# DINT-NSDI24/DINT

Hardware: AMD Instinct MI355X
Metric: Mtxn/s + p50/p99 batch latency, TATP (higher is better)
Workload: dtype u64

## Files before the change

### dint_amd/_lib.py

```python
from __future__ import annotations

import ctypes as C
import os

HERE = os.path.dirname(os.path.abspath(__file__))
LIB_PATH = os.environ.get("DINT_LIB_PATH") or os.path.join(HERE, "libdint.so")

ABI_VERSION = 5
FLAG_KV_ROUNDS, FLAG_COPY_STREAMS, FLAG_LOCK_SAME_KEY, FLAG_KV_NO_HOT, FLAG_INPUTS_READY = 1, 2, 4, 8, 16
MICRO_BATCH = 65536

SYMBOLS = [
    "dint_engine_create", "dint_engine_destroy", "dint_msg_size", "dint_last_error", "dint_submit",
    "dint_submit_device", "dint_sync", "dint_load_rows", "dint_populate", "dint_hash_size", "dint_dump_rows",
    "dint_read_locks", "dint_read_log", "dint_get_stats", "dint_reset", "dint_snapshot", "dint_restore",
    "dint_home_shard", "dint_bench_rand64", "dint_timing_enable", "dint_timing_read", "dint_kv_trace_read",
    "dint_submit_async", "dint_wait", "dint_alloc_pinned", "dint_free_pinned", "dint_engine_stream", "dint_max_pass",
    "dint_stream_wait", "dint_stream_signal", "dint_route_pack", "dint_route_unpack", "dint_submit_segments",
    "dint_log_drain", "dint_refuse", "dint_route_pack_multi", "dint_route_unpack_multi", "dint_bench_access", "dint_selftest",
    "dint_submit_segments_multi", "dint_submit_device_ahead", "dint_submit_segments_multi_ahead",
    "dint_log_drain_device", "dint_log_apply_device", "dint_state_digest", "dint_state_diff", "dint_state_repair",
    "dint_state_export", "dint_state_import", "dint_state_rehash", "dint_state_stats",
]
REHASH_DROP_LOCKS = 1
# ... 132 lines not shown
        "dint_route_pack_multi": (C.c_int, [C.POINTER(RouteItem), u32, u64, u64, vp]),
        "dint_route_unpack_multi": (C.c_int, [C.POINTER(RouteItem), u32, u64, vp]),
        "dint_submit_segments": (C.c_int, [vp, vp, u32, u32, u64, vp, u64, vp]),
        "dint_submit_segments_multi": (C.c_int, [C.POINTER(SegmentsItem), u32, vp]),
        "dint_submit_segments_multi_ahead": (C.c_int, [C.POINTER(SegmentsItem), u32, C.POINTER(SegmentsItem), vp]),
        "dint_log_drain": (i64, [vp, vp, u64, C.POINTER(u64)]),
        "dint_refuse": (C.c_int, [u32, vp, u32, vp]),
        "dint_log_drain_device": (i64, [vp, vp, u64, C.POINTER(u64), vp]),
        "dint_log_apply_device": (C.c_int, [vp, vp, u64, u32, C.POINTER(ApplyStats)]),
        "dint_state_digest": (C.c_int, [vp, C.POINTER(TableDigest), u32, vp]),
        "dint_state_diff": (i64, [vp, vp, vp, u64, C.POINTER(DiffStats), vp]),
        "dint_state_repair": (C.c_int, [vp, vp, u64, C.POINTER(RepairStats), vp]),
        "dint_state_export": (C.c_int, [vp, u32, u32, vp, u64, C.POINTER(ImageStats), vp]),
        "dint_state_import": (C.c_int, [vp, vp, u64, C.POINTER(ImageStats), vp]),
        "dint_state_rehash": (C.c_int, [vp, C.POINTER(vp), u32, u32, C.POINTER(RehashStats), vp]),
        "dint_state_stats": (C.c_int, [vp, C.POINTER(TableStats), u32, vp]),
        "dint_log_classify_host": (C.c_int, [vp, u64, vp, vp]),
        "dint_state_row_hash_host": (u64, [u64, u32, u32, vp, u32]),
        "dint_state_digest_host": (C.c_int, [u32, vp, vp, vp, u32, u64, C.POINTER(TableDigest)]),
        "dint_state_diff_host": (i64, [u32, u64, u32, vp, vp, vp, u64, vp, vp, vp, u64, vp, u64, C.POINTER(DiffStats)]),
        "dint_state_image_check_host": (C.c_int, [vp, u64]),
        "dint_state_stats_image_host": (C.c_int, [vp, u64, C.POINTER(TableStats), u32]),
        "dint_state_rehash_place_host": (i64, [vp, u64, u64, u32, u32, vp, vp, vp]),
    }
    for name, (res, args) in sig.items():
        f = getattr(L, name)
        f.restype, f.argtypes = res, args
    _lib = L
    return L


def check(rc: int) -> int:
    if rc < 0:
        raise DintError(f"dint error {rc}: {load().dint_last_error().decode(errors='replace')}")
    return rc
```

### dint_amd/csrc/dint_kv.h

```cpp
#pragma once
#include <cstdlib>
#include <utility>
#include <vector>

#include "dint_kernels.h"
#include "dint_kv_core.h"
#include "state_image.h"

#define DINT_KV_MAX_TABLES 5
#define DINT_KV_CTL_BYTES (64 + 24 * KV_NLISTS)
#define DINT_KV_TRACE_WORDS ((size_t)DINT_KV_PMAX * 16 + 16 * 8192)
#define DINT_KV_LOAD_OP 0xF0u

struct kv_dev {
  kv_tab tab[DINT_KV_MAX_TABLES];
  dint_mod mod[DINT_KV_MAX_TABLES];
  dint_mod lockmod[DINT_KV_MAX_TABLES];
  uint32_t gk_base[DINT_KV_MAX_TABLES];
  uint32_t n_tables;
  uint32_t shard_index, shard_count;
  uint32_t same_key;
};

struct dint_kv_knobs {
  uint32_t coarse_load = 512;
  uint32_t cap = 0;
  uint32_t lcap = 1024;
  uint32_t cap_mult = 64;
  uint32_t rpt = 0;
  uint32_t no_bm = 0;
  uint32_t hot_min = 0;
  uint32_t no_split = 0;
  uint32_t split_min = 65;
  uint32_t split_target = 384;
  uint32_t one_big_kernel = 0;
  uint32_t workers = 96;
  uint32_t part_first = 0;
  uint32_t sb_split_min = 65;
  uint32_t sb_npmax = 128;
  uint32_t sb_workers = 130;
  uint32_t sb_late_grid = 32;
  uint32_t residency = 0;
  uint32_t no_fuse = 0;
  uint32_t no_ahead = 0;
  uint32_t late_grid = 8;
  uint32_t exp_no_late = 0;
  uint32_t late_fat = 0;
  uint32_t late_big = 0;
};

struct dint_kv {
  uint32_t workload = 0;
  uint32_t n_tables = 0;
  uint32_t val_size = 0;
  int force_rounds = 0;
  uint64_t hash_size[DINT_KV_MAX_TABLES] = {0, 0, 0, 0, 0};
  kv_dev h{};
  kv_dev *d_dev = nullptr;
  uint8_t *d_ctl = nullptr;
  uint64_t *d_trace = nullptr;
  size_t entry_bytes[DINT_KV_MAX_TABLES] = {0, 0, 0, 0, 0};
  dint_kv_knobs knobs;
};

static inline uint32_t dint_kv_cap_mult() {
  const char *v = getenv("DINT_KV_CAP_MULT");
  const unsigned long m = v && *v ? strtoul(v, nullptr, 10) : 64ul;
  return (uint32_t)(m < 2 ? 2 : m > 256 ? 256 : m);
}
int dint_kv_create(dint_kv *kv, uint32_t workload, uint64_t n_rows, dint_shard shard, uint32_t pool_entries = 0,
                   uint32_t flags = 0);
void dint_kv_destroy(dint_kv *kv);
std::vector<std::pair<void *, size_t>> dint_kv_regions(dint_kv *kv);
// ... 132 lines not shown
```

### dint_amd/csrc/k_kv.hip

```cpp
#include "k_kv_dev.h"

dint_kv_fmt dint_kv_format(uint32_t workload) {
  switch (workload) {
    case DINT_WL_STORE: return {53, 0, 0xFFFFFFFFu, 1, 9, 49, 40};
    case DINT_WL_TATP: return {55, 1, 2, 3, 11, 51, 40};
    default: return {23, 1, 2, 3, 11, 19, 8};
  }
}


static inline uint32_t kv_pick_coarse(uint32_t n, uint32_t load) {
  uint64_t c = ((uint64_t)n + load - 1) / load;
  if (c < 1) c = 1;
  if (c > DINT_KV_CMAX) c = DINT_KV_CMAX;
  return (uint32_t)c;
}
static uint32_t kv_env(const char *name, uint32_t dflt) {
  const char *v = getenv(name);
  return v && *v ? (uint32_t)strtoul(v, nullptr, 10) : dflt;
}
static dint_kv_knobs kv_read_knobs() {
  dint_kv_knobs k;
  k.coarse_load = std::min(8192u, std::max(64u, kv_env("DINT_KV_COARSE_LOAD", KVB_T)));
  k.cap = kv_env("DINT_KV_CAP", 0);
  k.lcap = std::min(KVR_LCAP, kv_env("DINT_KV_LCAP", KVR_LCAP));
  k.cap_mult = dint_kv_cap_mult();
  k.rpt = kv_env("DINT_KV_RPT", 0);
  k.no_bm = kv_env("DINT_KV_NO_BM", 0);
  k.hot_min = kv_env("DINT_KV_HOT_MIN", 0);
  k.no_split = kv_env("DINT_KV_NO_SPLIT", 0);
  k.split_min = std::max(65u, kv_env("DINT_KV_SPLIT_MIN", 65u));
  k.split_target = std::min(448u, std::max(8u, kv_env("DINT_KV_SPLIT_TARGET", 384u)));
  k.one_big_kernel = kv_env("DINT_KV_ONE_BIG_KERNEL", 0);
  k.no_ahead = kv_env("DINT_KV_NO_AHEAD", 0);
  k.no_fuse = kv_env("DINT_KV_NO_FUSE", 0);
  k.sb_split_min = kv_env("DINT_KV_SB_SPLIT_MIN", 65u);
  k.sb_late_grid = std::max(1u, std::min(KVB_GRID, kv_env("DINT_KV_SB_LATE_GRID", 32u)));
  k.sb_npmax = std::max(2u, std::min(KSB_NPMAX, kv_env("DINT_KV_SB_NPMAX", 128u)));
  k.sb_workers = kv_env("DINT_KV_SB_WORKERS", k.sb_npmax + 2u);
  if (k.sb_workers) k.sb_workers = std::max(k.sb_workers, k.sb_npmax + 2u);
  k.workers = std::min(1024u, std::max(KVR_NPMAX + 2u, kv_env("DINT_KV_WORKERS", KVW_GRID)));
  k.part_first = kv_env("DINT_KV_PART_FIRST", 0) & 1u;
  k.late_grid = std::min(KVB_GRID, std::max(1u, kv_env("DINT_KV_LATE_GRID", 8u)));
  k.late_big = kv_env("DINT_KV_LATE_BIG", 0);
  k.exp_no_late = kv_env("DINT_EXP_NO_LATE", 0);
  k.late_fat = kv_env("DINT_KV_LATE_FAT", 0);
// ... 104 lines not shown
  kv_multi_args M, N;
  memset(&M, 0, sizeof M);
  uint32_t n_total = 0;
  for (uint32_t k = 0; k < n_eng; k++) n_total += p[k].n;
  const uint32_t rpt = kv_pick_rpt(n_total, p[0].kv->knobs);
  for (uint32_t k = 0; k < n_eng; k++) kv_fill_pass(M.e[k], p[k].d_req, p[k].d_rep, p[k].n, *p[k].kv, p[k].log, p[k].s, 0, p[k].view, KV_TB * rpt);
  uint32_t next_rpt = 0;
  if (next) {
    uint32_t nmax = 0;
    for (uint32_t k = 0; k < n_eng; k++) nmax = std::max(nmax, next[k].n);
    next_rpt = kv_pick_rpt_ahead(nmax, p[0].kv->knobs);
    memset(&N, 0, sizeof N);
    for (uint32_t k = 0; k < n_eng; k++) {
      dint_scratch sn = next[k].s;
      sn.kvs.pass_no = p[k].s.kvs.pass_no + 1;
      sn.pass_seq = p[k].s.pass_seq + 1 >= 0x3FFFFFFFu ? 1u : p[k].s.pass_seq + 1;
      kv_fill_pass(N.e[k], next[k].d_req, next[k].d_rep, next[k].n, *next[k].kv, next[k].log, sn, 0, next[k].view, KVB_T * next_rpt);
    }
  }
  launch_kv_dispatch(p[0].kv->workload, M, n_eng, rpt, st, nullptr, p[0].kv->knobs, part_done, next ? &N : nullptr, next_rpt);
}
bool dint_kv_multi_ahead_ok(const dint_kv &kv) { return dint_kv_ahead_ok(kv, 0) && !kv.knobs.no_fuse; }

__global__ void __launch_bounds__(256)
k_home_kv(const uint8_t *__restrict__ req, uint32_t n, const kv_dev *__restrict__ kv, dint_kv_fmt f,
          uint8_t *__restrict__ home) {
  const uint32_t i = blockIdx.x * 256u + threadIdx.x;
  if (i >= n) return;
  const uint8_t *m = req + (size_t)i * f.msg;
  const uint32_t table = f.table == 0xFFFFFFFFu ? 0 : m[f.table];
  if (table >= kv->n_tables) { home[i] = 0xFF; return; }
  const uint64_t g = dint_fastmod(dint_hash_key(ld_u64(m + f.key)), kv->mod[table]);
  home[i] = (uint8_t)(g % (kv->shard_count ? kv->shard_count : 1));
}
void dint_launch_home_kv(const void *d_req, uint32_t n, const dint_kv &kv, uint8_t *d_home, hipStream_t st) {
  if (n == 0) return;
  hipLaunchKernelGGL(k_home_kv, dim3((n + 255) / 256), dim3(256), 0, st, (const uint8_t *)d_req, n, kv.d_dev,
                     dint_kv_format(kv.workload), d_home);
}

int dint_kv_create(dint_kv *kv, uint32_t workload, uint64_t n_rows, dint_shard shard, uint32_t pool_entries,
                   uint32_t flags) {
  *kv = dint_kv();
  kv->workload = workload;
  kv->h.same_key = (workload == DINT_WL_TATP && (flags & DINT_FLAG_LOCK_SAME_KEY)) ? 1 : 0;
  uint64_t hs[DINT_KV_MAX_TABLES] = {0, 0, 0, 0, 0};
// ... 27 lines not shown
    if (hs[t] == 0) hs[t] = 1;
    kv->hash_size[t] = hs[t];
    kv_tab &tb = kv->h.tab[t];
    tb.n_local = (hs[t] + count - 1) / count;
    const uint64_t pool = pool_entries ? pool_entries : tb.n_local / 4 + 4096;
    if (pool > 0xFFFFFFF0ull || gk + tb.n_local > 0xFFFFFFF0ull) return DINT_EINVAL;
    tb.pool_cap = (uint32_t)pool;
    tb.stride = stride;
    tb.val_size = kv->val_size;
    kv->entry_bytes[t] = (size_t)(tb.n_local + tb.pool_cap) * stride;
    if (hipMalloc((void **)&tb.entries, kv->entry_bytes[t]) != hipSuccess) return DINT_ENOMEM;
    if (hipMemset(tb.entries, 0, kv->entry_bytes[t]) != hipSuccess) return DINT_EHIP;
    if (hipMalloc((void **)&tb.pool_next, (size_t)tb.pool_cap * 4) != hipSuccess) return DINT_ENOMEM;
    hipMemset(tb.pool_next, 0, (size_t)tb.pool_cap * 4);
    uint8_t *ctl = kv->d_ctl + DINT_KV_CTL_BYTES * t;
    tb.pool_top = (uint32_t *)ctl;
    tb.free_head = (unsigned long long *)(ctl + 64);
    tb.pend_head = (unsigned long long *)(ctl + 64 + 8 * KV_NLISTS);
    kv->h.mod[t] = dint_make_mod(hs[t]);
    kv->h.lockmod[t] = dint_make_mod(4 * hs[t]);
    kv->h.gk_base[t] = (uint32_t)gk;
    gk += tb.n_local;
  }
  kv->knobs = kv_read_knobs();
  {
    int dev = 0;
    (void)hipGetDevice(&dev);
    const int res = workload == DINT_WL_STORE ? kv_piece_residency<DINT_WL_STORE>(dev)
                    : workload == DINT_WL_TATP ? kv_piece_residency<DINT_WL_TATP>(dev) : kv_piece_residency<DINT_WL_SMALLBANK>(dev);
    kv->knobs.residency = (uint32_t)std::max(res, 0);
    if (workload == DINT_WL_SMALLBANK) {
      if (res < (int)(KSB_NPMAX + 2u + 32u)) kv->knobs.sb_split_min = 0;
    } else {
      if (res < 2 * (int)(KVR_NPMAX + 2u)) kv->knobs.no_split = 1;
      kv->knobs.workers = std::max(KVR_NPMAX + 2u, std::min(kv->knobs.workers, (uint32_t)std::max(res, 0) / 2u));
    }
  }
  if (getenv("DINT_KV_TRACE")) {
    if (hipMalloc((void **)&kv->d_trace, (size_t)DINT_KV_TRACE_WORDS * 8) != hipSuccess) return DINT_ENOMEM;
    hipMemset(kv->d_trace, 0, (size_t)DINT_KV_TRACE_WORDS * 8);
  }
  if (hipMalloc((void **)&kv->d_dev, sizeof(kv_dev)) != hipSuccess) return DINT_ENOMEM;
  if (hipMemcpy(kv->d_dev, &kv->h, sizeof(kv_dev), hipMemcpyHostToDevice) != hipSuccess) return DINT_EHIP;
  return 0;
}

void dint_kv_destroy(dint_kv *kv) {
// ... 133 lines not shown
```

### dint_amd/csrc/k_kv_dev.h

```cpp
#pragma once
#include <algorithm>
#include <cstdlib>
#include <cstring>
#include <utility>
#include <vector>

#include "../../include/dint_abi.h"
#include "dint_kv.h"
#define KVB_SORT_INLINE
#include "dint_bins.h"

template <int WL> struct Fmt;
template <> struct Fmt<DINT_WL_STORE> {
  static constexpr uint32_t MSG = 53, TYPE = 0, KEY = 1, VAL = 9, VER = 49, VS = 40;
  static constexpr bool HAS_TABLE = false;
  static constexpr uint32_t TABLE = 0;
};
template <> struct Fmt<DINT_WL_TATP> {
  static constexpr uint32_t MSG = 55, TYPE = 1, KEY = 3, VAL = 11, VER = 51, VS = 40;
  static constexpr bool HAS_TABLE = true;
  static constexpr uint32_t TABLE = 2;
};
template <> struct Fmt<DINT_WL_SMALLBANK> {
  static constexpr uint32_t MSG = 23, TYPE = 1, KEY = 3, VAL = 11, VER = 19, VS = 8;
// ... 475 lines not shown
    case DEL: if (st.exists) { st.exists = 0; st.toggles++; } else st.miss++; break;
    default: break;
  }
  return code;
}

__device__ static inline uint64_t shfl_u64(uint64_t v, int src) {
  const uint32_t hi = (uint32_t)__shfl((uint32_t)(v >> 32), src, 64), lo = (uint32_t)__shfl((uint32_t)v, src, 64);
  return ((uint64_t)hi << 32) | lo;
}
__device__ static inline uint64_t readlane_u64(uint64_t v, int l) {
  const uint32_t hi = (uint32_t)__builtin_amdgcn_readlane((uint32_t)(v >> 32), l);
  const uint32_t lo = (uint32_t)__builtin_amdgcn_readlane((uint32_t)v, l);
  return ((uint64_t)hi << 32) | lo;
}
__device__ static inline uint64_t run_mask(uint64_t heads, uint64_t le, uint64_t vm, int *head_lane) {
  const int hl = 63 - __clzll(heads & le);
  const uint64_t above = heads & ~le;
  const uint64_t next = above ? (above & (~above + 1ull)) : vm + 1ull;
  *head_lane = hl;
  return (next - 1ull) & ~((1ull << hl) - 1ull);
}

template <int WL>
__device__ static inline void kv_chunk(uint8_t *rep, bool valid, uint32_t idx, uint32_t gk, uint32_t kh, uint32_t type,
                                       uint32_t table, uint32_t q, uint64_t key_in, const kv_dev *kv,
                                       dint_dev_stats *__restrict__ stats, int force_rounds, bool last_chunk, const dint_view &V,
                                       uint64_t *tr = nullptr) {
  using F = Fmt<WL>;
  const int lane = (int)lane_id();
  const uint64_t lt = lanemask_lt(), le = lt | (1ull << lane);
  uint8_t *msg = rep + dint_view_off(V, idx, F::MSG);
  const uint64_t key = valid ? key_in : 0;
  const uint64_t bucket = valid ? (uint64_t)(gk - kv->gk_base[table]) : 0;

  const uint32_t gk_up = __shfl_up(gk, 1, 64), kh_up = __shfl_up(kh, 1, 64);
  const bool bhead = valid && (lane == 0 || gk_up != gk);
  const bool head = valid && (bhead || kh_up != kh);
  const uint64_t vm = __ballot(valid);
  const uint64_t bhm = __ballot(bhead), hm = __ballot(head);
  int hl = lane, bhl = lane;
  const uint64_t seg = valid ? run_mask(hm, le, vm, &hl) : 0;
  const uint64_t run = valid ? run_mask(bhm, le, vm, &bhl) : 0;

  uint32_t found = 0, link = 0, slot = 0, ver0 = 0, la0 = 0, lb0 = 0;
  kv_tab t;
  uint8_t *ie = nullptr;
// ... 1 lines not shown
  if (valid) {
    t = kv->tab[table];
    ie = kv_entry_ptr(t, bucket, KV_INLINE);
  }
  if (head) {
    kv_hdr_load(H, ie);
    if (WL == DINT_WL_SMALLBANK) {
      la0 = KV_LD(uint32_t, ie + KV_SB_LOCK_OFF + 8 * q); lb0 = KV_LD(uint32_t, ie + KV_SB_LOCK_OFF + 8 * q + 4);
    }
  }
  constexpr uint32_t NW = F::VS / 4;
  uint32_t w[NW];
#pragma unroll
  for (uint32_t k = 0; k < NW; k++) w[k] = 0;
  if (valid && kv_carries_val<WL>(type)) {
#pragma unroll
    for (uint32_t k = 0; k < NW; k++) w[k] = ld_u32(msg + F::VAL + 4 * k);
  }
  const uint64_t hkey = shfl_u64(key, hl);
  const uint64_t m_bad = __ballot(valid && !(key == hkey && (kv_simple_op<WL>(type) || kv_struct_op<WL>(type))));
  const uint64_t m_lockop = __ballot(valid && kv_lock_op<WL>(type));
  const uint64_t m_struct = __ballot(valid && kv_struct_op<WL>(type));
  const bool lkseg = head && (m_lockop & seg) != 0;
  bool lock_clash = false;
  bool my_clash = false;
#pragma unroll
  for (uint32_t k = 0; k < 4; k++) {
    const bool cl = __popcll(__ballot(lkseg && q == k) & run) > 1;
    lock_clash |= cl;
    my_clash |= cl && q == k;
  }
  if (WL == DINT_WL_TATP) lock_clash = false;
  const uint64_t m_stseg = __ballot(head && (m_struct & seg) != 0);
  bool simple = valid && (m_bad & run) == 0 && !lock_clash && __popcll(m_stseg & run) <= 1 && !force_rounds;
  const bool structural = (m_struct & seg) != 0;
  kv_stamp(tr, 4);
  int spec = -1;
  if (head) {
#pragma unroll
    for (int i = 0; i < 4; i++)
      if (spec < 0 && kv_valid(H, (uint32_t)i) && H.key[i] == key) spec = i;
  }
  spec = __shfl(spec, hl, 64);
  const bool spec_ld = valid && spec >= 0 && kv_may_get<WL>(type);
  if (spec_ld) {
    const uint8_t *sr = ie + KV_VAL_OFF + (uint32_t)spec * F::VS;
#pragma unroll
    for (uint32_t k = 0; k < NW; k++) w[k] = KV_LD(uint32_t, sr + 4 * k);
  }
  bool leader = head && simple;
  uint32_t dupf = 0;
  if (leader) {
    if (WL == DINT_WL_TATP) la0 = (H.lockw >> (8 * q)) & 0xFFu;
    const kv_where w = kv_locate(t, bucket, H, key);
    found = w.found; link = w.link; slot = w.slot; ver0 = w.ver;
    if (WL != DINT_WL_SMALLBANK && structural) dupf = kv_has_dup(t, bucket, H, key, w) | kv_pool_low(t);
  }
// ... 4 lines not shown
  uint32_t my_code = 0, my_ver = 0, my_get = 0;
  int my_src = -1;
  uint32_t fin_ver = ver0, fin_la = la0, fin_lb = lb0, nmiss = 0;
  int fin_src = -1;
  {
    const bool writer = simple && (WL == DINT_WL_STORE ? type == 1 : WL == DINT_WL_TATP ? (type == 12 || type == 13)
                                                                                       : (type == 4 || type == 5));
    const uint64_t m_wr = __ballot(writer && found) & seg;
    if (WL != DINT_WL_SMALLBANK) {
      const uint64_t wr_below = m_wr & lt;
      my_ver = ver0 + (uint32_t)__popcll(wr_below);
      my_src = wr_below ? 63 - __clzll(wr_below) : -1;
      fin_ver = ver0 + (uint32_t)__popcll(m_wr);
      fin_src = m_wr ? 63 - __clzll(m_wr) : -1;
      if (WL == DINT_WL_STORE) {
        my_code = type == 0 ? (found ? 3 : 7) : (found ? 5 : 7);
        my_get = (type == 0 && found) ? 1 : 0;
      } else {
        const uint64_t m_lk = __ballot(simple && kv_lock_op<WL>(type)) & seg;
        const uint64_t m_acq = __ballot(simple && type == 1);
        const uint64_t lk_below = m_lk & lt;
        uint32_t lock_seen = lk_below ? (uint32_t)((m_acq >> (63 - __clzll(lk_below))) & 1ull) : la0;
        if (m_lk) fin_la = (uint32_t)((m_acq >> (63 - __clzll(m_lk))) & 1ull);
        const uint64_t cm = __ballot(simple && my_clash && kv_lock_op<WL>(type));
        if (cm) {
          int seen = -1, fin = -1;
          uint32_t seen_at = 0, fin_at = 0;
          for (uint64_t mm = cm; mm; mm &= mm - 1) {
            const int l = __ffsll((unsigned long long)mm) - 1;
            const uint32_t oi = (uint32_t)__builtin_amdgcn_readlane(idx, l), og = (uint32_t)__builtin_amdgcn_readlane(gk, l);
            const uint32_t oq = (uint32_t)__builtin_amdgcn_readlane(q, l);
            const int acq = (uint32_t)__builtin_amdgcn_readlane(type, l) == 1;
            if (og == gk && oq == q) {
              if (oi < idx && (seen < 0 || oi > seen_at)) { seen_at = oi; seen = acq; }
              if (fin < 0 || oi > fin_at) { fin_at = oi; fin = acq; }
            }
          }
          if (simple && my_clash) {
            lock_seen = seen >= 0 ? (uint32_t)seen : la0;
            if (m_lk && fin >= 0) fin_la = (uint32_t)fin;
          }
        }
        nmiss = found ? 0 : (uint32_t)__popcll(__ballot(writer) & seg);
        switch (type) {
          case 0: my_code = found ? 4 : 6; my_get = found; break;
          case 1: my_code = lock_seen ? 8 : 7; break;
          case 2: my_code = 9; break;
          case 12: my_code = 15; break;
          default: my_code = 16; break;
        }
      }
      uint32_t fin_exists = found, fin_multi = 0, my_bail = 0;
      uint64_t stm = __ballot(leader && structural);
      while (stm) {
        const int L = __ffsll((unsigned long long)stm) - 1;
        stm &= stm - 1;
        const uint64_t sm = readlane_u64(seg, L);
        kv_rowst st;
        st.exists = (uint32_t)__builtin_amdgcn_readlane(found, L);
        st.ver = (uint32_t)__builtin_amdgcn_readlane(ver0, L);
        st.toggles = 0; st.miss = 0; st.bail = (uint32_t)__builtin_amdgcn_readlane(dupf, L); st.src = -1;
        for (uint64_t m = sm; m; m &= m - 1) {
          const int l = __ffsll((unsigned long long)m) - 1;
          const uint32_t op = (uint32_t)__builtin_amdgcn_readlane(type, l);
          uint32_t get = 0;
          const uint32_t ver_seen = st.ver;
          const int src_seen = st.src;
          const uint32_t code = kv_row_step<WL>(op, l, st, get);
          if (lane == l) {
            if (code) my_code = code;
            my_ver = ver_seen; my_src = src_seen; my_get = get;
          }
        }
        if (lane == L) {
          fin_exists = st.exists; fin_ver = st.ver; fin_src = st.src; nmiss = st.miss;
          fin_multi = st.toggles > 1;
          my_bail = st.bail;
        }
      }
      const uint64_t m_bail = __ballot(head && my_bail);
      if (m_bail & run) { simple = false; leader = false; }
      found = simple && structural ? (found | (fin_exists << 1) | (fin_multi << 2)) : found;
    } else {
      auto sb_step = [](uint32_t op, uint32_t fnd, uint32_t &la, uint32_t &lb, uint32_t &get, uint32_t &miss,
                        bool &wr) -> uint32_t {
        switch (op) {
          case 0: if (la == 0) { lb++; get = fnd; miss += !fnd; return 7; } return 8;
          case 1: if (la == 0 && lb == 0) { la++; get = fnd; miss += !fnd; return 9; } return 10;
          case 2: lb--; return 11;
          case 3: la--; return 12;
          case 4: wr = fnd; miss += !fnd; return 13;
          case 17: get = fnd; return 18;
          default: wr = fnd; miss += !fnd; return 14;
        }
      };
      const bool single = simple && seg == (1ull << lane);
      if (single) {
        bool wr = false;
        my_code = sb_step(type, found, fin_la, fin_lb, my_get, nmiss, wr);
        my_ver = ver0;
        if (wr) { fin_ver = ver0 + 1; fin_src = lane; }
      }
      uint64_t multi = __ballot(leader && !single);
// ... 32 lines not shown
      if (getting && my_src >= 0) w[k] = o;
    }
  }
  uint8_t *row = nullptr;
  if (simple) {
    row = kv_entry_ptr(t, bucket, link) + KV_VAL_OFF + slot * F::VS;
    if (my_get) {
      if (my_src < 0 && !(spec_ld && link == KV_INLINE && slot == (uint32_t)spec)) {
#pragma unroll
        for (uint32_t k = 0; k < NW; k++) w[k] = KV_LD(uint32_t, row + 4 * k);
      }
#pragma unroll
      for (uint32_t k = 0; k < NW; k++) st_u32(msg + F::VAL + 4 * k, w[k]);
      st_u32(msg + F::VER, my_ver);
    }
    msg[F::TYPE] = (uint8_t)my_code;
    if (!structural && (found & 1u) && seg_fin_src == lane) {
#pragma unroll
      for (uint32_t k = 0; k < NW; k++) KV_ST(uint32_t, row + 4 * k, w[k]);
      KV_ST(uint32_t, &kv_entry_hdr(t, bucket, link)->ver[slot], seg_fin_ver);
    }
  }
  kv_stamp(tr, 6);
  if (__ballot(leader && structural)) __builtin_amdgcn_fence(__ATOMIC_SEQ_CST, "workgroup");
  if (leader) {
    const uint32_t found0 = found & 1u, exists1 = structural ? (found >> 1) & 1u : found0;
    const bool redo = structural && found0 && exists1 && ((found >> 2) & 1u);
    if (found0 && exists1 && !redo) {
      if (structural && fin_src >= 0) {
        kv_copy_words(row, rep + dint_view_off(V, fin_idx, F::MSG) + F::VAL, F::VS);
        KV_ST(uint32_t, &kv_entry_hdr(t, bucket, link)->ver[slot], fin_ver);
      }
    } else if (found0 != exists1 || redo) {
      if (redo) {
        kv_apply<kv_dev_mem>(t, bucket, H, KV_ACT_DEL, key, nullptr, 0, blockIdx.x);
        __builtin_amdgcn_fence(__ATOMIC_SEQ_CST, "workgroup");
        kv_hdr_load(H, ie);
      }
      const kv_res r = kv_apply<kv_dev_mem>(t, bucket, H, exists1 ? KV_ACT_INS : KV_ACT_DEL, key,
                                            rep + dint_view_off(V, fin_idx, F::MSG) + F::VAL, fin_ver, blockIdx.x);
      if (exists1 && !r.ok) atomicAdd(&stats->pool_exhausted, 1ULL);
    }
    if (WL == DINT_WL_TATP && fin_la != la0) KV_ST(uint8_t, ie + KV_LOCKB_OFF + q, (uint8_t)fin_la);
    if (WL == DINT_WL_SMALLBANK && (fin_la != la0 || fin_lb != lb0)) {
      KV_ST(uint32_t, ie + KV_SB_LOCK_OFF + 8 * q, fin_la);
      KV_ST(uint32_t, ie + KV_SB_LOCK_OFF + 8 * q + 4, fin_lb);
    }
    if (nmiss) atomicAdd(&stats->missing_keys, (unsigned long long)nmiss);
  }
  kv_stamp(tr, 7);

  const bool rounds = valid && !simple;
  uint64_t rheads = __ballot(rounds && bhead);
  if (rheads) {
    const uint64_t m_rd = __ballot(valid && kv_pure_read<WL>(type));
    uint32_t pos = 0, maxlen = 0;
    while (rheads) {
      const int L = __ffsll((unsigned long long)rheads) - 1;
      rheads &= rheads - 1;
      const uint64_t rmask = readlane_u64(run, L);
      maxlen = max(maxlen, 2u * (uint32_t)__popcll(rmask & ~m_rd) + 1u);
      const bool mine = (rmask >> lane) & 1ull;
      for (uint64_t m = rmask & ~m_rd; m; m &= m - 1) {
        const int l = __ffsll((unsigned long long)m) - 1;
        const uint32_t oi = (uint32_t)__builtin_amdgcn_readlane(idx, l);
        if (mine && oi < idx) pos++;
      }
    }
    pos = 2u * pos + (kv_pure_read<WL>(type) ? 0u : 1u);
    for (uint32_t r = 0; r < maxlen; r++) {
      if (rounds && pos == r) kv_do_request<WL>(msg, type, table, q, bucket, kv, stats);
      __builtin_amdgcn_fence(__ATOMIC_SEQ_CST, "workgroup");
    }
  }
  if (!last_chunk) __builtin_amdgcn_fence(__ATOMIC_SEQ_CST, "workgroup");
  kv_stamp(tr, 8);
// ... 1242 lines not shown
        __syncthreads();
      }
    }
    }
    if (wtr && t == 0) { wtr[14] += nrounds; wtr[15] += 1; }
    KVB_STAMP(13);
    __builtin_amdgcn_fence(__ATOMIC_SEQ_CST, "workgroup");
    __syncthreads();
  }
#undef KVB_STAMP
}

#define KVR_LCAP 1024u
#define KVR_F 64u
#define KVR_NPMAX 64u
struct kvr_lds {
  uint4 rec[KVR_LCAP];
  uint32_t hist[KVR_F];
  uint32_t cur[KVR_F];
  uint32_t off[KVR_F + 1];
  uint32_t bigoff[KVR_F];
  uint2 chs[KVR_F];
  uint32_t nch;
  uint32_t cflag[KVR_F];
  uint64_t ckey[KVR_F], hrec[KVR_F];
};
__device__ static inline uint32_t kv_piece_of(uint32_t idx, uint32_t np, uint32_t inv_n) {
  const uint32_t p = (uint32_t)(((uint64_t)idx * np * inv_n) >> 32);
  return p < np ? p : np - 1;
}
#define KVQ_W 3u
enum : uint32_t { KVQ_SUB = 0, KVQ_PIECE = 1, KVQ_REM = 2, KVQ_SOLO = 3 };

__device__ static inline void kv_list_items(const kv_pass_args &A, uint32_t b, const kvr_lds &L, const uint2 *Sbig) {
  const uint32_t t = threadIdx.x & 63u;
  const uint2 bs = Sbig[t];
  uint32_t target = A.split_target;
  if (A.V.seg_cap) {
    uint32_t live = t < A.V.n_seg ? min(A.V.seg_cap, *(const uint32_t *)(A.V.cnt + (size_t)t * A.V.cnt_stride)) : 0u, tot;
    (void)wave_excl_scan_u32(live, &tot);
    if (tot < A.n) target = max(8u, (uint32_t)(((uint64_t)target * max(tot, 1u)) / A.n));
  }
  const uint32_t np0 = (bs.y + target - 1) / target;
  const bool hot = bs.y >= A.split_min && np0 <= A.np_max;
  const uint32_t np = hot ? np0 : 0u;
  const uint32_t nent = bs.y ? (np > 1 ? np + 1 : 1u) : 0u;
// ... 66 lines not shown
      uint4 q4[8];
#pragma unroll
      for (uint32_t j = 0; j < 8; j++) {
        const uint32_t k = k0 + j * NT + t;
        q4[j] = k < n_in ? recs[k] : make_uint4(0, 0, 0, 0);
      }
#pragma unroll
      for (uint32_t j = 0; j < 8; j++)
        if (k0 + j * NT + t < n_in) f(q4[j]);
    }
    for (uint32_t k0 = 0; k0 < novl; k0 += 8 * NT) {
      uint32_t b8[8];
#pragma unroll
      for (uint32_t j = 0; j < 8; j++) {
        const uint32_t k = k0 + j * NT + t;
        b8[j] = k < novl ? A.ovl[2 * (size_t)k + 1].x : KV_NONE;
      }
#pragma unroll
      for (uint32_t j = 0; j < 8; j++)
        if (b8[j] == coarse) f(A.ovl[2 * (size_t)(k0 + j * NT + t)]);
    }
  };
  auto big_rec = [&](uint64_t m) -> uint64_t { return ((m >> (sh + 6)) << sh) | (m & ((1ull << sh) - 1ull)); };
  for_each_record([&](const uint4 &r) {
    const uint64_t m = u4_meta(r);
    const uint32_t sub = (uint32_t)(m >> sh) & (KVR_F - 1);
    const uint32_t sub0 = (uint32_t)__builtin_amdgcn_readfirstlane((int)sub);
    const uint64_t same = __ballot(sub == sub0);
    if (sub != sub0) atomicAdd(&L.hist[sub], 1u);
    else if (lane == (uint32_t)__ffsll((unsigned long long)same) - 1) atomicAdd(&L.hist[sub], (uint32_t)__popcll(same));
    if (L.cflag[sub] == 0 && atomicCAS(&L.cflag[sub], 0u, 1u) == 0u) { L.ckey[sub] = u4_key(r); L.hrec[sub] = big_rec(m); }
  });
  __syncthreads();
  if (tr && t == 0) tr[2] = __builtin_amdgcn_s_memrealtime();
  if (wave == 0) {
    const uint32_t h = L.hist[lane];
    bool big = h > 64;
    uint32_t stot, sc = big ? 0u : h, soff = wave_excl_scan_u32(sc, &stot);
    if (stot > A.lcap) {
      big = h > 0; sc = 0; soff = 0; stot = 0;
    }
    uint32_t btot = 0, boff = 0, gbase = 0;
    if (__ballot(big)) {
      boff = wave_excl_scan_u32(big ? h : 0u, &btot);
      if (lane == 0) {
        gbase = atomicAdd(&A.big[0], btot);
        atomicAdd(&A.stats->big_bin_requests, (unsigned long long)btot);
      }
      gbase = (uint32_t)__builtin_amdgcn_readfirstlane((int)gbase);
    }
    L.off[lane] = soff;
    if (lane == 63) L.off[KVR_F] = stot;
    L.bigoff[lane] = big ? gbase + boff : KV_NONE;
    Sbig[lane] = make_uint2(big ? gbase + boff : 0u, big ? h : 0u);
    uint32_t lo = lane + 1, hi = KVR_F;
#pragma unroll
    for (int it = 0; it < 7; it++) {
      const uint32_t mid = min((lo + hi + 1) >> 1, KVR_F);
      const uint32_t v = (uint32_t)__shfl((int)soff, (int)(mid & (KVR_F - 1)), 64);
      const uint32_t om = mid == KVR_F ? stot : v;
      if (lo < hi) {
        if (om - soff <= 64u) lo = mid; else hi = mid - 1;
      }
    }
    uint32_t s = 0, nch = 0;
    while (s < KVR_F) {
      const uint32_t e = (uint32_t)__builtin_amdgcn_readlane((int)lo, (int)s);
      const uint32_t os = (uint32_t)__builtin_amdgcn_readlane((int)soff, (int)s);
      const uint32_t oe = e >= KVR_F ? stot : (uint32_t)__builtin_amdgcn_readlane((int)soff, (int)e);
      if (oe > os) {
        if (lane == 0) L.chs[nch] = make_uint2(os, oe);
        nch++;
      }
      s = e;
    }
    if (lane == 0) L.nch = nch;
    if (tr && lane == 0) { tr[14] = cnt; tr[15] = btot; tr[16] = nch; }
  }
  __syncthreads();
  if (tr && t == 0) tr[3] = __builtin_amdgcn_s_memrealtime();
  for_each_record([&](const uint4 &r) {
    const uint64_t m = u4_meta(r);
    const uint32_t sub = (uint32_t)(m >> sh) & (KVR_F - 1);
    const uint32_t sub0 = (uint32_t)__builtin_amdgcn_readfirstlane((int)sub);
    const uint64_t same = __ballot(sub == sub0);
    const int lead = __ffsll((unsigned long long)same) - 1;
    uint32_t pos = 0;
    if (sub != sub0) pos = atomicAdd(&L.cur[sub], 1u);
    else if ((int)lane == lead) pos = atomicAdd(&L.cur[sub], (uint32_t)__popcll(same));
    if (sub == sub0) pos = (uint32_t)__builtin_amdgcn_readlane((int)pos, lead) + (uint32_t)__popcll(same & lanemask_lt());
    const uint32_t bo = L.bigoff[sub];
    if (bo == KV_NONE) L.rec[L.off[sub] + pos] = r;
    else kv_st_agent(&A.ovf[bo + pos], big_rec(m));
  });
  asm volatile("s_waitcnt vmcnt(0)" ::: "memory");
  __syncthreads();
  if (tr && t == 0) tr[4] = __builtin_amdgcn_s_memrealtime();
  if (wave == NT / 64 - 1) kv_list_items(A, coarse, L, Sbig);
  const uint32_t nch = L.nch;
  for (uint32_t ch = wave; ch < nch; ch += NT / 64) {
    const uint2 ab = L.chs[ch];
    const uint32_t c = ab.y - ab.x;
    const bool has = lane < c;
    const uint4 r = has ? L.rec[ab.x + lane] : make_uint4(0, 0, 0, 0);
    const uint64_t key0 = u4_key(r), m = u4_meta(r);
    const uint32_t pay0 = kv_rec_pay(m);
    uint64_t w = ~0ull;
    if (has) w = ((m >> sh) << (15 + cut.ibits)) | ((uint64_t)pay_kh(pay0) << (6 + cut.ibits)) | ((uint64_t)((uint32_t)(m >> 16) & idx_mask) << 6) | lane;
    w = wave_sort_u64(w);
    uint64_t *ctr = (tr && ch == 0) ? tr + 2 : nullptr;
    if (ctr && lane == 0) tr[5] = __builtin_amdgcn_s_memrealtime();
    const bool valid = lane < c;
    const int src = (int)((uint32_t)w & 63u);
    const uint64_t key = shfl_u64(key0, src);
    const uint32_t pay = (uint32_t)__shfl((int)pay0, src, 64);
    const uint32_t gk = kv_cut_gk((uint32_t)(w >> (15 + cut.ibits)), coarse, cut), kh = (uint32_t)(w >> (6 + cut.ibits)) & 511u;
    const uint32_t idx = (uint32_t)(w >> 6) & idx_mask;
    kv_chunk<WL>(A.rep, valid, valid ? idx : 0, gk, kh, pay_type(pay), valid ? kv_table_of(kv, gk) : 0, pay_q(pay), key, kv, A.stats,
                 A.force_flags & 1, true, A.V, ctr);
  }
}

template <int WL>
__device__ __forceinline__ static void kv_resolve_role(const kv_pass_args &A, uint32_t b, kv_dev &Skv, uint8_t *Lraw, uint2 *Sbig) {
  constexpr uint32_t NT = KVB_T;
  const uint32_t t = threadIdx.x;
  uint64_t *tr = A.trace ? A.trace + 32 * (size_t)b : nullptr;
  if (tr && t == 0) tr[0] = __builtin_amdgcn_s_memrealtime();
  static_assert(sizeof(kv_dev) / 4 <= NT, "one word of the table descriptors per thread");
  const uint4 *__restrict__ recs = A.kbins + (size_t)b * A.cap;
  const uint4 r0 = t < A.cap ? recs[t] : make_uint4(0, 0, 0, 0);
  const uint4 r1 = t + NT < A.cap ? recs[t + NT] : make_uint4(0, 0, 0, 0);
  const uint32_t kvw = t < sizeof(kv_dev) / 4 ? ((const uint32_t *)A.kv)[t] : 0u;
  const uint32_t cnt = A.bin_cnt[b];
  if (t < sizeof(kv_dev) / 4) ((uint32_t *)&Skv)[t] = kvw;
  if (t < KVR_F) {
    Sbig[t] = make_uint2(0u, 0u);
    kvr_lds &L = *(kvr_lds *)Lraw;
    L.hist[t] = 0; L.cur[t] = 0; L.cflag[t] = 0;
  }
  if (b == 0) {
    if (t < 16) A.big_z[t] = 0;
// ... 1361 lines not shown
```

### include/dint_driver.h

```cpp
#ifndef DINT_DRIVER_H
#define DINT_DRIVER_H

#include <stdint.h>

#ifdef __cplusplus
extern "C" {
#endif

#define DINT_N_SHARDS 3

typedef struct dint_driver dint_driver_t;

typedef struct dint_driver_config {
  uint32_t workload;
  uint32_t n_clients;
  uint64_t n_rows;
  uint32_t first_client;
  uint32_t key_dist;
  double zipf_theta;
  uint32_t reserved[8];
} dint_driver_config;

typedef struct dint_driver_stats {
  uint64_t txns;
// ... 80 lines not shown
int dint_lock_gclient_read_batch(dint_lock_gclient_t *c, void *host);
int dint_lock_gclient_get_stats(dint_lock_gclient_t *c, dint_fasst_client_stats *out);

int dint_log_classify_host(const void *records, uint64_t n, const uint8_t *exists0, uint8_t *types_out);

struct dint_table_digest;
struct dint_diff_stats;
uint64_t dint_state_row_hash_host(uint64_t key, uint32_t ver, uint32_t table, const void *val, uint32_t val_size);
int dint_state_digest_host(uint32_t table, const uint64_t *keys, const uint32_t *vers, const void *vals, uint32_t val_size,
                           uint64_t n, struct dint_table_digest *out);
int64_t dint_state_diff_host(uint32_t table, uint64_t hash_size, uint32_t val_size, const uint64_t *a_keys, const uint32_t *a_vers,
                             const void *a_vals, uint64_t na, const uint64_t *b_keys, const uint32_t *b_vers, const void *b_vals,
                             uint64_t nb, void *records, uint64_t cap, struct dint_diff_stats *out);


int dint_state_image_check_host(const void *image, uint64_t bytes);

struct dint_table_stats;
int dint_state_stats_image_host(const void *image, uint64_t bytes, struct dint_table_stats *out, uint32_t cap_tables);

int64_t dint_state_rehash_place_host(const uint64_t *keys, uint64_t n, uint64_t hash_size, uint32_t shard_index, uint32_t shard_count,
                                     uint64_t *bucket_out, uint32_t *link_out, uint32_t *slot_out);

#ifdef __cplusplus
}
#endif
#endif
```

Measured before the change: 2983.

## Add lean fast path in kv_chunk and dynamic chunk scheduling in coarse kernel

Adds a TRY_LEAN template path to kv_chunk. When a warp has no bad, structural or forced-round ops and no same-segment lock clashes, it skips the per-queue clash ballots, the structural and bail ballots, the fence and the rounds setup; it is enabled for every workload except SmallBank. The coarse partition kernel now skips the wave-merged histogram and cursor atomics when the block has few records, and records the big-sub key only on the overflow path. Chunks are handed out through an LDS atomic ticket instead of a fixed stride. The packing rule is moved into shared host/device helpers with a host export, adding a lean-detection ballot and extra code paths that could mis-handle edge cases.

```diff
diff --git a/dint_amd/_lib.py b/dint_amd/_lib.py
--- a/dint_amd/_lib.py
+++ b/dint_amd/_lib.py
@@ -178,6 +178,7 @@
         "dint_state_image_check_host": (C.c_int, [vp, u64]),
         "dint_state_stats_image_host": (C.c_int, [vp, u64, C.POINTER(TableStats), u32]),
         "dint_state_rehash_place_host": (i64, [vp, u64, u64, u32, u32, vp, vp, vp]),
+        "dint_kv_chunk_pack_host": (C.c_int, [vp, vp, vp]),
     }
     for name, (res, args) in sig.items():
         f = getattr(L, name)
diff --git a/dint_amd/csrc/dint_kv.h b/dint_amd/csrc/dint_kv.h
--- a/dint_amd/csrc/dint_kv.h
+++ b/dint_amd/csrc/dint_kv.h
@@ -3,6 +3,7 @@
 #include <utility>
 #include <vector>
 
+#include "../../include/dint_abi.h"
 #include "dint_kernels.h"
 #include "dint_kv_core.h"
 #include "state_image.h"
@@ -49,6 +50,45 @@
   uint32_t late_big = 0;
 };
 
+static inline uint32_t kv_pick_coarse(uint32_t n, uint32_t load) {
+  uint64_t c = ((uint64_t)n + load - 1) / load;
+  if (c < 1) c = 1;
+  if (c > DINT_KV_CMAX) c = DINT_KV_CMAX;
+  return (uint32_t)c;
+}
+#define KV_PACK_SUBS 64u
+#define KV_PACK_CHUNK 64u
+#define KV_PACK_WAVES 8u
+static inline uint32_t kv_default_coarse_load(uint32_t workload) { (void)workload; return 512u; }
+template <class OffAt>
+__host__ __device__ static inline uint32_t kv_pack_next(uint32_t l, uint32_t off_l, uint32_t stot, OffAt &&off_at) {
+  uint32_t lo = l + 1, hi = KV_PACK_SUBS;
+#pragma unroll
+  for (int it = 0; it < 7; it++) {
+    const uint32_t m0 = (lo + hi + 1) >> 1, mid = m0 < KV_PACK_SUBS ? m0 : KV_PACK_SUBS;
+    const uint32_t v = off_at(mid & (KV_PACK_SUBS - 1));
+    const uint32_t om = mid == KV_PACK_SUBS ? stot : v;
+    if (lo < hi) {
+      if (om - off_l <= KV_PACK_CHUNK) lo = mid; else hi = mid - 1;
+    }
+  }
+  return lo;
+}
+template <class NextAt, class OffAt, class Emit>
+__host__ __device__ static inline uint32_t kv_pack_walk(uint32_t stot, NextAt &&next_at, OffAt &&off_at, Emit &&emit) {
+  uint32_t s = 0, nch = 0;
+  while (s < KV_PACK_SUBS) {
+    const uint32_t e = next_at(s), os = off_at(s);
+    const uint32_t oe = e >= KV_PACK_SUBS ? stot : off_at(e);
+    if (oe > os) {
+      emit(nch, os, oe);
+      nch++;
+    }
+    s = e;
+  }
+  return nch;
+}
+
 struct dint_kv {
   uint32_t workload = 0;
   uint32_t n_tables = 0;
diff --git a/dint_amd/csrc/k_kv.hip b/dint_amd/csrc/k_kv.hip
--- a/dint_amd/csrc/k_kv.hip
+++ b/dint_amd/csrc/k_kv.hip
@@ -1,4 +1,5 @@
 #include "k_kv_dev.h"
+#include "../../include/dint_driver.h"
 
 dint_kv_fmt dint_kv_format(uint32_t workload) {
   switch (workload) {
@@ -9,19 +10,13 @@
 }
 
 
-static inline uint32_t kv_pick_coarse(uint32_t n, uint32_t load) {
-  uint64_t c = ((uint64_t)n + load - 1) / load;
-  if (c < 1) c = 1;
-  if (c > DINT_KV_CMAX) c = DINT_KV_CMAX;
-  return (uint32_t)c;
-}
 static uint32_t kv_env(const char *name, uint32_t dflt) {
   const char *v = getenv(name);
   return v && *v ? (uint32_t)strtoul(v, nullptr, 10) : dflt;
 }
-static dint_kv_knobs kv_read_knobs() {
+static dint_kv_knobs kv_read_knobs(uint32_t workload) {
   dint_kv_knobs k;
-  k.coarse_load = std::min(8192u, std::max(64u, kv_env("DINT_KV_COARSE_LOAD", KVB_T)));
+  k.coarse_load = std::min(8192u, std::max(64u, kv_env("DINT_KV_COARSE_LOAD", kv_default_coarse_load(workload))));
   k.cap = kv_env("DINT_KV_CAP", 0);
   k.lcap = std::min(KVR_LCAP, kv_env("DINT_KV_LCAP", KVR_LCAP));
   k.cap_mult = dint_kv_cap_mult();
@@ -172,6 +167,18 @@
 }
 bool dint_kv_multi_ahead_ok(const dint_kv &kv) { return dint_kv_ahead_ok(kv, 0) && !kv.knobs.no_fuse; }
 
+extern "C" int dint_kv_chunk_pack_host(const uint32_t *hist, uint32_t *first, uint32_t *last) {
+  if (!hist || !first || !last) return DINT_EINVAL;
+  uint32_t off[KV_PACK_SUBS + 1], next[KV_PACK_SUBS];
+  off[0] = 0;
+  for (uint32_t l = 0; l < KV_PACK_SUBS; l++) off[l + 1] = off[l] + (hist[l] > KV_PACK_CHUNK ? 0u : hist[l]);
+  const uint32_t stot = off[KV_PACK_SUBS];
+  auto off_at = [&](uint32_t l) { return off[l]; };
+  for (uint32_t l = 0; l < KV_PACK_SUBS; l++) next[l] = kv_pack_next(l, off[l], stot, off_at);
+  return (int)kv_pack_walk(stot, [&](uint32_t s) { return next[s]; }, off_at,
+                           [&](uint32_t c, uint32_t os, uint32_t oe) { first[c] = os; last[c] = oe; });
+}
+
 __global__ void __launch_bounds__(256)
 k_home_kv(const uint8_t *__restrict__ req, uint32_t n, const kv_dev *__restrict__ kv, dint_kv_fmt f,
           uint8_t *__restrict__ home) {
@@ -245,7 +252,7 @@
     kv->h.gk_base[t] = (uint32_t)gk;
     gk += tb.n_local;
   }
-  kv->knobs = kv_read_knobs();
+  kv->knobs = kv_read_knobs(workload);
   {
     int dev = 0;
     (void)hipGetDevice(&dev);
diff --git a/dint_amd/csrc/k_kv_dev.h b/dint_amd/csrc/k_kv_dev.h
--- a/dint_amd/csrc/k_kv_dev.h
+++ b/dint_amd/csrc/k_kv_dev.h
@@ -521,7 +521,7 @@
   return (next - 1ull) & ~((1ull << hl) - 1ull);
 }
 
-template <int WL>
+template <int WL, bool TRY_LEAN = false>
 __device__ static inline void kv_chunk(uint8_t *rep, bool valid, uint32_t idx, uint32_t gk, uint32_t kh, uint32_t type,
                                        uint32_t table, uint32_t q, uint64_t key_in, const kv_dev *kv,
                                        dint_dev_stats *__restrict__ stats, int force_rounds, bool last_chunk, const dint_view &V,
@@ -569,17 +569,25 @@
   const uint64_t m_lockop = __ballot(valid && kv_lock_op<WL>(type));
   const uint64_t m_struct = __ballot(valid && kv_struct_op<WL>(type));
   const bool lkseg = head && (m_lockop & seg) != 0;
+  bool lean = false;
+  if (TRY_LEAN) {
+    lean = !force_rounds && (m_bad | m_struct) == 0;
+    if (lean && hm != bhm && m_lockop) lean = __ballot(valid && __popcll(__ballot(lkseg) & run) > 1) == 0;
+  }
   bool lock_clash = false;
   bool my_clash = false;
-#pragma unroll
-  for (uint32_t k = 0; k < 4; k++) {
-    const bool cl = __popcll(__ballot(lkseg && q == k) & run) > 1;
-    lock_clash |= cl;
-    my_clash |= cl && q == k;
+  uint64_t m_stseg = 0;
+  if (!lean) {
+#pragma unroll
+    for (uint32_t k = 0; k < 4; k++) {
+      const bool cl = __popcll(__ballot(lkseg && q == k) & run) > 1;
+      lock_clash |= cl;
+      my_clash |= cl && q == k;
+    }
+    m_stseg = __ballot(head && (m_struct & seg) != 0);
   }
   if (WL == DINT_WL_TATP) lock_clash = false;
-  const uint64_t m_stseg = __ballot(head && (m_struct & seg) != 0);
-  bool simple = valid && (m_bad & run) == 0 && !lock_clash && __popcll(m_stseg & run) <= 1 && !force_rounds;
+  bool simple = valid && (lean || ((m_bad & run) == 0 && !lock_clash && __popcll(m_stseg & run) <= 1 && !force_rounds));
   const bool structural = (m_struct & seg) != 0;
   kv_stamp(tr, 4);
   int spec = -1;
@@ -630,7 +638,8 @@
         const uint64_t lk_below = m_lk & lt;
         uint32_t lock_seen = lk_below ? (uint32_t)((m_acq >> (63 - __clzll(lk_below))) & 1ull) : la0;
         if (m_lk) fin_la = (uint32_t)((m_acq >> (63 - __clzll(m_lk))) & 1ull);
-        const uint64_t cm = __ballot(simple && my_clash && kv_lock_op<WL>(type));
+        uint64_t cm = 0;
+        if (!lean) cm = __ballot(simple && my_clash && kv_lock_op<WL>(type));
         if (cm) {
           int seen = -1, fin = -1;
           uint32_t seen_at = 0, fin_at = 0;
@@ -659,7 +668,8 @@
         }
       }
       uint32_t fin_exists = found, fin_multi = 0, my_bail = 0;
-      uint64_t stm = __ballot(leader && structural);
+      uint64_t stm = 0;
+      if (!lean) stm = __ballot(leader && structural);
       while (stm) {
         const int L = __ffsll((unsigned long long)stm) - 1;
         stm &= stm - 1;
@@ -686,7 +696,8 @@
           my_bail = st.bail;
         }
       }
-      const uint64_t m_bail = __ballot(head && my_bail);
+      uint64_t m_bail = 0;
+      if (!lean) m_bail = __ballot(head && my_bail);
       if (m_bail & run) { simple = false; leader = false; }
       found = simple && structural ? (found | (fin_exists << 1) | (fin_multi << 2)) : found;
     } else {
@@ -765,7 +776,7 @@
     }
   }
   kv_stamp(tr, 6);
-  if (__ballot(leader && structural)) __builtin_amdgcn_fence(__ATOMIC_SEQ_CST, "workgroup");
+  if (!lean && __ballot(leader && structural)) __builtin_amdgcn_fence(__ATOMIC_SEQ_CST, "workgroup");
   if (leader) {
     const uint32_t found0 = found & 1u, exists1 = structural ? (found >> 1) & 1u : found0;
     const bool redo = structural && found0 && exists1 && ((found >> 2) & 1u);
@@ -794,7 +805,8 @@
   kv_stamp(tr, 7);
 
   const bool rounds = valid && !simple;
-  uint64_t rheads = __ballot(rounds && bhead);
+  uint64_t rheads = 0;
+  if (!lean) rheads = __ballot(rounds && bhead);
   if (rheads) {
     const uint64_t m_rd = __ballot(valid && kv_pure_read<WL>(type));
     uint32_t pos = 0, maxlen = 0;
@@ -2083,6 +2095,7 @@
   uint32_t bigoff[KVR_F];
   uint2 chs[KVR_F];
   uint32_t nch;
+  uint32_t tick;
   uint32_t cflag[KVR_F];
   uint64_t ckey[KVR_F], hrec[KVR_F];
 };
@@ -2195,14 +2208,18 @@
     }
   };
   auto big_rec = [&](uint64_t m) -> uint64_t { return ((m >> (sh + 6)) << sh) | (m & ((1ull << sh) - 1ull)); };
+  const bool merge_subs = cnt > 2 * NT;
   for_each_record([&](const uint4 &r) {
     const uint64_t m = u4_meta(r);
     const uint32_t sub = (uint32_t)(m >> sh) & (KVR_F - 1);
+    if (!merge_subs) {
+      atomicAdd(&L.hist[sub], 1u);
+      return;
+    }
     const uint32_t sub0 = (uint32_t)__builtin_amdgcn_readfirstlane((int)sub);
     const uint64_t same = __ballot(sub == sub0);
     if (sub != sub0) atomicAdd(&L.hist[sub], 1u);
     else if (lane == (uint32_t)__ffsll((unsigned long long)same) - 1) atomicAdd(&L.hist[sub], (uint32_t)__popcll(same));
-    if (L.cflag[sub] == 0 && atomicCAS(&L.cflag[sub], 0u, 1u) == 0u) { L.ckey[sub] = u4_key(r); L.hrec[sub] = big_rec(m); }
   });
   __syncthreads();
   if (tr && t == 0) tr[2] = __builtin_amdgcn_s_memrealtime();
@@ -2226,27 +2243,14 @@
     if (lane == 63) L.off[KVR_F] = stot;
     L.bigoff[lane] = big ? gbase + boff : KV_NONE;
     Sbig[lane] = make_uint2(big ? gbase + boff : 0u, big ? h : 0u);
-    uint32_t lo = lane + 1, hi = KVR_F;
-#pragma unroll
-    for (int it = 0; it < 7; it++) {
-      const uint32_t mid = min((lo + hi + 1) >> 1, KVR_F);
-      const uint32_t v = (uint32_t)__shfl((int)soff, (int)(mid & (KVR_F - 1)), 64);
-      const uint32_t om = mid == KVR_F ? stot : v;
-      if (lo < hi) {
-        if (om - soff <= 64u) lo = mid; else hi = mid - 1;
-      }
-    }
-    uint32_t s = 0, nch = 0;
-    while (s < KVR_F) {
-      const uint32_t e = (uint32_t)__builtin_amdgcn_readlane((int)lo, (int)s);
-      const uint32_t os = (uint32_t)__builtin_amdgcn_readlane((int)soff, (int)s);
-      const uint32_t oe = e >= KVR_F ? stot : (uint32_t)__builtin_amdgcn_readlane((int)soff, (int)e);
-      if (oe > os) {
-        if (lane == 0) L.chs[nch] = make_uint2(os, oe);
-        nch++;
-      }
-      s = e;
-    }
+    static_assert(KVR_F == KV_PACK_SUBS && NT / 64 == KV_PACK_WAVES, "the packing rule is written for 64 subs and 8 waves");
+    auto soff_at = [&](uint32_t l) { return (uint32_t)__shfl((int)soff, (int)l, 64); };
+    const uint32_t lo = kv_pack_next(lane, soff, stot, soff_at);
+    const uint32_t nch = kv_pack_walk(
+        stot, [&](uint32_t s) { return (uint32_t)__builtin_amdgcn_readlane((int)lo, (int)s); },
+        [&](uint32_t s) { return (uint32_t)__builtin_amdgcn_readlane((int)soff, (int)s); },
+        [&](uint32_t c, uint32_t os, uint32_t oe) { if (lane == 0) L.chs[c] = make_uint2(os, oe); });
+    if (lane == 0) L.tick = NT / 64;
     if (lane == 0) L.nch = nch;
     if (tr && lane == 0) { tr[14] = cnt; tr[15] = btot; tr[16] = nch; }
   }
@@ -2255,23 +2259,31 @@
   for_each_record([&](const uint4 &r) {
     const uint64_t m = u4_meta(r);
     const uint32_t sub = (uint32_t)(m >> sh) & (KVR_F - 1);
-    const uint32_t sub0 = (uint32_t)__builtin_amdgcn_readfirstlane((int)sub);
-    const uint64_t same = __ballot(sub == sub0);
-    const int lead = __ffsll((unsigned long long)same) - 1;
     uint32_t pos = 0;
-    if (sub != sub0) pos = atomicAdd(&L.cur[sub], 1u);
-    else if ((int)lane == lead) pos = atomicAdd(&L.cur[sub], (uint32_t)__popcll(same));
-    if (sub == sub0) pos = (uint32_t)__builtin_amdgcn_readlane((int)pos, lead) + (uint32_t)__popcll(same & lanemask_lt());
+    if (!merge_subs) {
+      pos = atomicAdd(&L.cur[sub], 1u);
+    } else {
+      const uint32_t sub0 = (uint32_t)__builtin_amdgcn_readfirstlane((int)sub);
+      const uint64_t same = __ballot(sub == sub0);
+      const int lead = __ffsll((unsigned long long)same) - 1;
+      if (sub != sub0) pos = atomicAdd(&L.cur[sub], 1u);
+      else if ((int)lane == lead) pos = atomicAdd(&L.cur[sub], (uint32_t)__popcll(same));
+      if (sub == sub0) pos = (uint32_t)__builtin_amdgcn_readlane((int)pos, lead) + (uint32_t)__popcll(same & lanemask_lt());
+    }
     const uint32_t bo = L.bigoff[sub];
-    if (bo == KV_NONE) L.rec[L.off[sub] + pos] = r;
-    else kv_st_agent(&A.ovf[bo + pos], big_rec(m));
+    if (bo == KV_NONE) {
+      L.rec[L.off[sub] + pos] = r;
+    } else {
+      kv_st_agent(&A.ovf[bo + pos], big_rec(m));
+      if (L.cflag[sub] == 0 && atomicCAS(&L.cflag[sub], 0u, 1u) == 0u) { L.ckey[sub] = u4_key(r); L.hrec[sub] = big_rec(m); }
+    }
   });
   asm volatile("s_waitcnt vmcnt(0)" ::: "memory");
   __syncthreads();
   if (tr && t == 0) tr[4] = __builtin_amdgcn_s_memrealtime();
   if (wave == NT / 64 - 1) kv_list_items(A, coarse, L, Sbig);
   const uint32_t nch = L.nch;
-  for (uint32_t ch = wave; ch < nch; ch += NT / 64) {
+  for (uint32_t ch = wave; ch < nch;) {
     const uint2 ab = L.chs[ch];
     const uint32_t c = ab.y - ab.x;
     const bool has = lane < c;
@@ -2289,8 +2301,12 @@
     const uint32_t pay = (uint32_t)__shfl((int)pay0, src, 64);
     const uint32_t gk = kv_cut_gk((uint32_t)(w >> (15 + cut.ibits)), coarse, cut), kh = (uint32_t)(w >> (6 + cut.ibits)) & 511u;
     const uint32_t idx = (uint32_t)(w >> 6) & idx_mask;
-    kv_chunk<WL>(A.rep, valid, valid ? idx : 0, gk, kh, pay_type(pay), valid ? kv_table_of(kv, gk) : 0, pay_q(pay), key, kv, A.stats,
-                 A.force_flags & 1, true, A.V, ctr);
+    kv_chunk<WL, WL != DINT_WL_SMALLBANK>(A.rep, valid, valid ? idx : 0, gk, kh, pay_type(pay), valid ? kv_table_of(kv, gk) : 0, pay_q(pay),
+                                          key, kv, A.stats, A.force_flags & 1, true, A.V, ctr);
+    if (nch <= NT / 64) break;
+    uint32_t nx = 0;
+    if (lane == 0) nx = atomicAdd(&L.tick, 1u);
+    ch = (uint32_t)__builtin_amdgcn_readfirstlane((int)nx);
   }
 }
 
diff --git a/include/dint_driver.h b/include/dint_driver.h
--- a/include/dint_driver.h
+++ b/include/dint_driver.h
@@ -126,6 +126,8 @@
 int64_t dint_state_rehash_place_host(const uint64_t *keys, uint64_t n, uint64_t hash_size, uint32_t shard_index, uint32_t shard_count,
                                      uint64_t *bucket_out, uint32_t *link_out, uint32_t *slot_out);
 
+int dint_kv_chunk_pack_host(const uint32_t *hist, uint32_t *first, uint32_t *last);
+
 #ifdef __cplusplus
 }
 #endif
```

Result: no change. 3010, median of 6 (+0.9%).
